# szcompressor/SZ3

Hardware: AMD Instinct MI355X
Metric: compression throughput GB/s + ratio at fixed abs errBound, 512^3 f32 (higher is better)
Workload: dtype f32; 1 GPU; C2: 3D float32 512x512x512 synthetic field per GPU, Lorenzo predictor, abs errBound=0.001, device-resident in -> device-resident Huffman payload; parallelism=slab1, algo=HIP_LORENZO(16), exchange=none (one rank)

## Files before the change

### include/sz3hip_debug.h

```cpp
#ifndef SZ3HIP_DEBUG_H
#define SZ3HIP_DEBUG_H

enum sz3hip_dbg {
    SZ3HIP_DBG_CB_COMPACT_IN_WG = 1,
    SZ3HIP_DBG_K1_LAB_NO_HIST = 1,
    SZ3HIP_DBG_DEC_MULTI_SYM = 2,
    SZ3HIP_DBG_K1_NO_CODE_STORES = 2,
    SZ3HIP_DBG_BLKDEC_FORCE_RETRY = 4,
    SZ3HIP_DBG_K1_V4_NO_STENCIL = 4,
    SZ3HIP_DBG_K1_NO_Q16 = 8,
    SZ3HIP_DBG_BLKDEC_LOCAL_EXPANDED = 16,
    SZ3HIP_DBG_K1_V4_NO_PREFETCH = 16,
    SZ3HIP_DBG_PACK_LAB_NO_STORES = 16,
    SZ3HIP_DBG_K1_NO_MARCH = 32,
    SZ3HIP_DBG_K1_NO_NARROW = 64,
    SZ3HIP_DBG_INTERP_NO_VEC = 128,
    SZ3HIP_DBG_K1_NO_WIDTH_SPEC = 256,
    SZ3HIP_DBG_DEC_NO_FUSED_X = 512,
    SZ3HIP_DBG_PACK_LAB_ONE_UNIT = 512,
    SZ3HIP_DBG_CB_ONE_CLASS = 1024,
    SZ3HIP_DBG_K1_NO_FUSED = 2048,
    SZ3HIP_DBG_BLK_RANK_3_LAUNCHES = 2048,
    SZ3HIP_DBG_BLK_SIDE_8_LAUNCHES = 2048,
    SZ3HIP_DBG_K1_NO_XCD_ORDER = 4096,
    SZ3HIP_DBG_CB_NO_SPEC_WIDE = 4096,
    SZ3HIP_DBG_INTERP_HIST_BIG = 8192,
    SZ3HIP_DBG_BLK_OFF = 16384,
    SZ3HIP_DBG_PACK_OLD = 32768,
    SZ3HIP_DBG_BLKDEC_GROUPS_3 = 32768,
    SZ3HIP_DBG_CB_NO_SAMPLED = 65536,
    SZ3HIP_DBG_BLKDEC_PER_FRONT = 65536,
    SZ3HIP_DBG_CTX_NO_MEMORY = 131072,
    SZ3HIP_DBG_CB_SERIAL_MERGE = 262144,
    SZ3HIP_DBG_DEC_NO_STORES = 524288,
    SZ3HIP_DBG_DEC_DIRECT_STORES = 1048576,
    SZ3HIP_DBG_DEC_NO_HALF = 2097152,
    SZ3HIP_DBG_INTERP_LEVELS_ANY_SIZE = 4194304,
    SZ3HIP_DBG_K1_NO_SAMP_IN_LAUNCH = 4194304,
    SZ3HIP_DBG_BLKDEC_BLOCK_PER_WAVE = 8388608,
    SZ3HIP_DBG_K1_Q16_PLAIN_STORES = 8388608,
    SZ3HIP_DBG_K1_NO_DEFER_FOLD = 16777216,
    SZ3HIP_DBG_PACK_NO_SEG_BITS = 33554432,
    SZ3HIP_DBG_BLK_FIT_TILES = 67108864,
    SZ3HIP_DBG_BLK_1D_WAVE_PER_BLOCK = 134217728,
    SZ3HIP_DBG_CTX_NO_PUBLISH_ZERO = 268435456,
    SZ3HIP_DBG_INTERP_HANDOVER_IN_PLACE = 536870912,
    SZ3HIP_DBG_DEC_CARRY_PASS = 536870912,
    SZ3HIP_DBG_BLK_NO_EXIT = 1073741824,
    SZ3HIP_DBG_BLK_NO_SELECT = -2147483647 - 1
};

enum sz3hip_dbg2 {
    SZ3HIP_DBG2_PACK_SCAN_LAUNCH = 1
};

#endif
```

### sz3_amd/__init__.py

```python
import contextlib
import ctypes as C
import enum
import os

import numpy as np

_HERE = os.path.dirname(os.path.abspath(__file__))
LIB_PATH = os.environ.get("SZ3HIP_LIB") or os.path.join(_HERE, "libsz3hip.so")

EB_ABS, EB_REL, EB_PSNR, EB_L2NORM, EB_ABS_AND_REL, EB_ABS_OR_REL = range(6)
ALGO_LORENZO_REG, ALGO_INTERP_LORENZO, ALGO_INTERP, ALGO_NOPRED, ALGO_LOSSLESS = range(5)
ALGO_HIP_LORENZO = 16
ALGO_HIP_INTERP = 17
INTERP_ALGO_LINEAR, INTERP_ALGO_CUBIC = 0, 1
SZ_FLOAT, SZ_DOUBLE = 0, 1


class Dbg(enum.IntFlag):
    CB_COMPACT_IN_WG = 1
    K1_LAB_NO_HIST = 1
    DEC_MULTI_SYM = 2
    K1_NO_CODE_STORES = 2
    BLKDEC_FORCE_RETRY = 4
    K1_V4_NO_STENCIL = 4
# ... 11 lines not shown
    K1_NO_FUSED = 2048
    BLK_RANK_3_LAUNCHES = 2048
    BLK_SIDE_8_LAUNCHES = 2048
    K1_NO_XCD_ORDER = 4096
    CB_NO_SPEC_WIDE = 4096
    INTERP_HIST_BIG = 8192
    BLK_OFF = 16384
    PACK_OLD = 32768
    BLKDEC_GROUPS_3 = 32768
    CB_NO_SAMPLED = 65536
    BLKDEC_PER_FRONT = 65536
    CTX_NO_MEMORY = 131072
    CB_SERIAL_MERGE = 262144
    DEC_NO_STORES = 524288
    DEC_DIRECT_STORES = 1048576
    DEC_NO_HALF = 2097152
    INTERP_LEVELS_ANY_SIZE = 4194304
    K1_NO_SAMP_IN_LAUNCH = 4194304
    BLKDEC_BLOCK_PER_WAVE = 8388608
    K1_Q16_PLAIN_STORES = 8388608
    K1_NO_DEFER_FOLD = 16777216
    PACK_NO_SEG_BITS = 33554432
    BLK_FIT_TILES = 67108864
    BLK_1D_WAVE_PER_BLOCK = 134217728
    CTX_NO_PUBLISH_ZERO = 268435456
    INTERP_HANDOVER_IN_PLACE = 536870912
    DEC_CARRY_PASS = 536870912
    BLK_NO_EXIT = 1073741824
    BLK_NO_SELECT = 2147483648


class Dbg2(enum.IntFlag):
    PACK_SCAN_LAUNCH = 1


class SZ3HipError(RuntimeError):
    def __init__(self, code, msg):
        super().__init__("sz3hip error %d: %s" % (code, msg))
        self.code = code


class _CConfig(C.Structure):
    _fields_ = [
        ("N", C.c_int32), ("dims", C.c_uint64 * 4), ("num", C.c_uint64),
        ("cmprAlgo", C.c_uint8), ("errorBoundMode", C.c_uint8),
        ("absErrorBound", C.c_double), ("relErrorBound", C.c_double),
        ("psnrErrorBound", C.c_double), ("l2normErrorBound", C.c_double),
        ("openmp", C.c_uint8), ("quantbinCnt", C.c_int32), ("blockSize", C.c_int32),
        ("predDim", C.c_uint8), ("dataType", C.c_uint8),
        ("lorenzo", C.c_uint8), ("lorenzo2", C.c_uint8), ("regression", C.c_uint8), ("regression2", C.c_uint8),
        ("interpAlgo", C.c_uint8), ("interpDirection", C.c_uint8),
        ("interpAnchorStride", C.c_int32), ("interpAlpha", C.c_double), ("interpBeta", C.c_double),
    ]


class _CTunerReport(C.Structure):
    _fields_ = [("ran", C.c_int32), ("use_interp", C.c_int32), ("sample_block_size", C.c_uint64), ("n_filtered", C.c_uint64),
                ("n_blocks", C.c_uint64), ("profiling", C.c_int32), ("interpAlgo", C.c_int32), ("interpDirection", C.c_int32),
                ("speculated", C.c_int32), ("interpAlpha", C.c_double), ("interpBeta", C.c_double), ("est_bytes", C.c_double * 8)]


class _CStats(C.Structure):
    _fields_ = [("n", C.c_uint64), ("n_value_outliers", C.c_uint64), ("n_delta_outliers", C.c_uint64),
                ("n_chunks", C.c_uint64), ("bitstream_bytes", C.c_uint64), ("payload_bytes", C.c_uint64),
                ("n_symbols", C.c_uint32), ("max_code_len", C.c_uint32),
                ("narrow_codes", C.c_uint32), ("reserved", C.c_uint32)]
# ... 992 lines not shown
```

### sz3_amd/csrc/sz3hip_kernels.h

```cpp
#ifndef SZ3HIP_KERNELS_H
#define SZ3HIP_KERNELS_H
#include <hip/hip_runtime.h>
#include <stdint.h>
#include "sz3hip_format.h"
#include "../../include/sz3hip_debug.h"

struct szk_lattice {
    double recip, two_eb, eb;
    float recip_f, two_eb_f, eb_lo_f;
};
static inline szk_lattice szk_make_lattice(double eb) {
    szk_lattice l;
    l.eb = eb;
    l.two_eb = 2.0 * eb;
    l.recip = 1.0 / l.two_eb;
    l.recip_f = (float)l.recip;
    l.two_eb_f = (float)l.two_eb;
    float e = (float)eb;
    if ((double)e > eb) e = __builtin_nextafterf(e, 0.0f);
    l.eb_lo_f = e;
    return l;
}

#define SZK_K1_GRID 2048u
// ... 6 lines not shown
    uint64_t n_total;
    uint32_t allow;
};

struct szk_cb_info;
#define SZK_SAMP_UNITS 1024u
#define SZK_SAMP_ROLES 128u
#define SZK_SAMP_MIN_ELEMS (1ull << 22)
#define SZK_SAMP_SEEN_LEN 16u
#define SZK_SAMP_WORDS 512u
#define SZK_SAMP_TICKET 320u
#define SZK_SAMP_LENS 384u
#define SZK_SAMP_READY 448u
struct szk_samp {
    uint32_t *words;
    uint32_t *enc;
    uint8_t *lens;
    szk_cb_info *info;
};
struct szk_k1_params {
    uint64_t d[4];
    szk_lattice lat;
    uint32_t radius;
    uint32_t dbg;
    szk_mode mode;
    uint64_t out_cap;
    uint64_t *hist;
    uint32_t *hist_partial;
    uint64_t *n_vout, *n_dout;
    uint64_t *vout_idx, *dout_idx;
    void *vout_val, *dout_val;
    void *prof_ev0, *prof_ev1;
    uint32_t wide16;
    uint32_t *range;
    int hint_narrow;
    const uint8_t *spec_lens;
    uint16_t *seg_bits;
    uint32_t *seg_made;
    int seg_expected;
    int assumed_narrow;
    int hint_q16;
    int assumed_q16;
    uint32_t *q16_flag;
    int defer_fold;
    uint32_t fold_rows;
    int range_kept;
    int fuse;
    int fused;
    const uint32_t *fuse_enc;
    const szk_cb_info *fuse_info;
    uint32_t *fuse_slots;
    uint64_t fuse_cap_words;
    uint32_t *seg_base;
    uint32_t *fuse_flag;
    uint32_t fuse_geom[4];
    szk_samp samp;
    int samp_in_launch;
};

struct szk_cb_info {
    uint32_t n_symbols, max_len, sym_min, sym_count;
    uint32_t win_lo, reserved;
    uint32_t esc_sym, pad0;
    uint64_t ts[12];
    uint32_t first_code[SZH_MAX_LEN + 2];
};
// ... 397 lines not shown
```

### sz3_amd/csrc/sz3hip_kernels.hip

```cpp
#include <hip/hip_runtime.h>
#include <cstddef>
#include <stdint.h>
#include <type_traits>
#include <mutex>
#include <utility>
#include <vector>
#include "sz3hip_format.h"
#include "sz3hip_kernels.h"

#include "sz3hip_devutil.h"

template <typename T>
__global__ __launch_bounds__(256) void k_minmax(const T *__restrict__ in, uint64_t n, double *partial) {
    double mn = INFINITY, mx = -INFINITY;
    bool has_nan = false;
    for (uint64_t i = (uint64_t)blockIdx.x * blockDim.x + threadIdx.x; i < n; i += (uint64_t)gridDim.x * blockDim.x) {
        double v = (double)in[i];
        if (v < mn) mn = v;
        if (v > mx) mx = v;
        has_nan |= (v != v);
    }
    (void)has_nan;
#pragma unroll
    for (int d = WAVE / 2; d > 0; d >>= 1) {
// ... 797 lines not shown
                if (MODE == 1 || MODE == 4) hist_add_ranged(p.hist, p.range, sym, (unsigned long long)v);
                else atomicAdd((unsigned long long *)&p.hist[sym], (unsigned long long)v);
            }
        }
    }
}

#define NARROW_BINS 256
template <typename T> struct NarrowCtx {
    using B = typename Lattice<T>::B;
    using OQV = typename std::conditional<sizeof(T) == 4, uint32_t, uint64_t>::type;
    const T *in;
    uint8_t *codes8;
    const szk_k1_params *p;
    uint32_t d0, d1, d2;
    uint64_t plane, vol;
    uint32_t *lh;
    const uint8_t *s_len;
    uint16_t *seg_bits;
    uint64_t *oq_idx;
    OQV *oq_val;
    uint32_t oq_n;
    int lane;
    const uint32_t *s_enc;
    uint32_t *stage;
    uint32_t *slot;
    uint32_t slot_base;
    uint32_t slot_w;
    uint32_t st_cnt;
    uint32_t *seg_base;
    const uint32_t *samp_words;
    uint32_t *s_have;
    uint32_t have_len;
};
#define FUSE_STAGE_WORDS(TY) ((TY) * 128 + 32 + 8)
static inline uint32_t fuse_slot_words(uint32_t ty, uint64_t d1, uint64_t d2) {
    return (uint32_t)((d1 < ty ? d1 : ty) * 128u * (d2 < MARCH_TZ ? d2 : MARCH_TZ) + 32u);
}
template <typename T>
__device__ __forceinline__ void narrow_oq_flush(NarrowCtx<T> &c) {
    c.oq_n = (uint32_t)__builtin_amdgcn_readfirstlane((int)c.oq_n);
    if (c.oq_n == 0) return;
    const szk_k1_params &p = *c.p;
    const unsigned long long act = __ballot(1);
    const uint32_t nact = (uint32_t)__popcll(act), rank = (uint32_t)__popcll(act & ((1ull << c.lane) - 1ull));
    unsigned long long base = 0;
    if (rank == 0) base = atomicAdd((unsigned long long *)p.n_vout, (unsigned long long)c.oq_n);
    const uint32_t blo = (uint32_t)__builtin_amdgcn_readfirstlane((int)(uint32_t)base);
    const uint32_t bhi = (uint32_t)__builtin_amdgcn_readfirstlane((int)(uint32_t)(base >> 32));
    const unsigned long long b0 = ((unsigned long long)bhi << 32) | blo;
    for (uint32_t k = rank; k < c.oq_n; k += nact) {
        const unsigned long long pos = b0 + k;
        if (pos < p.out_cap) {
            p.vout_idx[pos] = c.oq_idx[k];
            if (sizeof(T) == 4) reinterpret_cast<uint32_t *>(p.vout_val)[pos] = (uint32_t)c.oq_val[k];
            else reinterpret_cast<uint64_t *>(p.vout_val)[pos] = c.oq_val[k];
        }
    }
    c.oq_n = 0;
}
template <typename T>
__device__ __forceinline__ void narrow_rare(NarrowCtx<T> &c, uint64_t gi, const typename QTraits<T>::UQ (&delta)[4], uint32_t tmask, uint32_t badmask) {
    using Q = typename QTraits<T>::Q;
    using OQV = typename NarrowCtx<T>::OQV;
    const szk_k1_params &p = *c.p;
    constexpr uint32_t OQ = MarchLds<1, false>::OQ;
// ... 8 lines not shown
                }
                pd++;
            }
    }
#pragma unroll
    for (int i = 0; i < 4; i++) {
        const bool is_vout = (badmask >> i) & 1u;
        const unsigned long long vm = __ballot(is_vout);
        if (vm) {
            c.oq_n = (uint32_t)__builtin_amdgcn_readfirstlane((int)c.oq_n);
            if (c.oq_n + WAVE > OQ) narrow_oq_flush(c);
            if (is_vout) {
                const uint32_t slot = c.oq_n + (uint32_t)__popcll(vm & ((1ull << c.lane) - 1ull));
                c.oq_idx[slot] = gi + i;
                const T raw = c.in[gi + i];
                OQV bits = 0;
                memcpy(&bits, &raw, sizeof(T));
                c.oq_val[slot] = bits;
            }
            c.oq_n += (uint32_t)__popcll(vm);
        }
    }
    {
        const uint32_t cnt = (uint32_t)__popc(tmask & 15u);
        const unsigned long long b0 = __ballot(cnt & 1u), b1 = __ballot(cnt & 2u), b2 = __ballot(cnt & 4u), any = b0 | b1 | b2;
        if (any && c.lane == __ffsll((long long)any) - 1)
            hist_add_ranged(p.hist, p.range, 0u, (unsigned long long)(__popcll(b0) + 2 * __popcll(b1) + 4 * __popcll(b2)));
    }
}
template <typename T> __device__ __forceinline__ bool samp_take(const T *__restrict__ in, const szk_lattice &latp, uint32_t d0, uint32_t d1, uint32_t d2, uint32_t *words, uint32_t role, uint32_t *s_h);
__device__ __forceinline__ void samp_book(const szk_samp &sp, uint32_t radius, uint8_t *pool);
#define SAMP_POOL_BYTES (SZK_CB_SMALL_SYMS * 28 + 256)
template <typename T, typename PUT>
__device__ __forceinline__ bool samp_poll(NarrowCtx<T> &c, bool spin, PUT put) {
    volatile uint32_t *s_have = c.s_have;
    const uint32_t wv = (uint32_t)__builtin_amdgcn_readfirstlane((int)(threadIdx.x / WAVE));
    if (wv != 0) {
        uint32_t h = (uint32_t)__builtin_amdgcn_readfirstlane((int)*s_have);
        if (!h) {
            if (!spin) return false;
            do {
                __builtin_amdgcn_s_sleep(16);
                h = (uint32_t)__builtin_amdgcn_readfirstlane((int)*s_have);
            } while (!h);
        }
        __builtin_amdgcn_fence(__ATOMIC_ACQUIRE, "workgroup");
        c.have_len = 1;
        return true;
    }
    uint32_t r = __hip_atomic_load(const_cast<uint32_t *>(c.samp_words) + SZK_SAMP_READY, __ATOMIC_RELAXED, __HIP_MEMORY_SCOPE_AGENT);
    r = (uint32_t)__builtin_amdgcn_readfirstlane((int)r);
    if (!r) {
        if (!spin) return false;
        do {
            __builtin_amdgcn_s_sleep(32);
            r = __hip_atomic_load(const_cast<uint32_t *>(c.samp_words) + SZK_SAMP_READY, __ATOMIC_RELAXED, __HIP_MEMORY_SCOPE_AGENT);
            r = (uint32_t)__builtin_amdgcn_readfirstlane((int)r);
        } while (!r);
    }
    const uint32_t w = __hip_atomic_load(const_cast<uint32_t *>(c.samp_words) + SZK_SAMP_LENS + c.lane, __ATOMIC_RELAXED, __HIP_MEMORY_SCOPE_AGENT);
#pragma unroll
    for (int j = 0; j < 4; j++) put(4u * (uint32_t)c.lane + j, (w >> (8 * j)) & 0xFFu);
    __builtin_amdgcn_fence(__ATOMIC_RELEASE, "workgroup");
    __builtin_amdgcn_wave_barrier();
    if (c.lane == 0) *s_have = 1u;
    c.have_len = 1;
    return true;
}
template <typename T, int NW, int TY> struct NarrowPlane {
    Quad<T> rq[NW][TY + 1];
    T rl[NW][TY + 1];
    bool rok[NW][TY + 1];
};
template <typename T>
__device__ __forceinline__ void fuse_sweep(NarrowCtx<T> &c, uint32_t nw) {
    uint32_t *out = c.slot + c.slot_w;
    auto sweep = [&](uint32_t i) {
        const uint2 wv = *reinterpret_cast<const uint2 *>(&c.stage[i]);
        *reinterpret_cast<uint2 *>(&c.stage[i]) = make_uint2(0u, 0u);
#if defined(LAB_FUSE) && (LAB_FUSE & 32)
        *reinterpret_cast<unsigned long long *>(&out[i]) = (unsigned long long)wv.x | ((unsigned long long)wv.y << 32);
#else
        __builtin_nontemporal_store((unsigned long long)wv.x | ((unsigned long long)wv.y << 32), reinterpret_cast<unsigned long long *>(&out[i]));
#endif
    };
    const uint32_t i0 = 2u * (uint32_t)c.lane;
    if (i0 < nw) sweep(i0);
    if (i0 + 2u * WAVE < nw) sweep(i0 + 2u * WAVE);
    if (nw > 4u * WAVE)
        for (uint32_t i = i0 + 4u * WAVE; i < nw; i += 2u * WAVE) sweep(i);
}
template <typename T>
__device__ __forceinline__ void fuse_flush_lines(NarrowCtx<T> &c) {
#if defined(LAB_FUSE) && (LAB_FUSE & 4)
    const uint32_t nfl = 0;
    c.st_cnt &= 31u;
#else
    const uint32_t nfl = c.st_cnt & ~31u;
#endif
// ... 449 lines not shown
    for (int bnn = threadIdx.x; bnn < HIST_WIN; bnn += 256) {
        const int t = bnn - (HIST_WIN / 2 - 127);
        row[bnn] = (t >= 0 && t < 255) ? lh[t * 4] + lh[t * 4 + 1] + lh[t * 4 + 2] + lh[t * 4 + 3] : 0u;
    }
}

#define Q16_LIM 4095.0f
typedef float v2f32 __attribute__((ext_vector_type(2)));
typedef unsigned short v2u16 __attribute__((ext_vector_type(2)));
__device__ __forceinline__ uint32_t pk_sub16(uint32_t a, uint32_t b) {
    return __builtin_bit_cast(uint32_t, (v2u16)(__builtin_bit_cast(v2u16, a) - __builtin_bit_cast(v2u16, b)));
}
__device__ __forceinline__ uint32_t pk_add16(uint32_t a, uint32_t b) {
    return __builtin_bit_cast(uint32_t, (v2u16)(__builtin_bit_cast(v2u16, a) + __builtin_bit_cast(v2u16, b)));
}
__device__ __forceinline__ uint32_t pk_min16(uint32_t a, uint32_t b) {
    return __builtin_bit_cast(uint32_t, __builtin_elementwise_min(__builtin_bit_cast(v2u16, a), __builtin_bit_cast(v2u16, b)));
}
__device__ __forceinline__ uint32_t pk_max16(uint32_t a, uint32_t b) {
    return __builtin_bit_cast(uint32_t, __builtin_elementwise_max(__builtin_bit_cast(v2u16, a), __builtin_bit_cast(v2u16, b)));
}
__device__ __forceinline__ uint32_t pk_lo16(uint32_t a, uint32_t b) { return __builtin_amdgcn_perm(b, a, 0x05040100u); }
__device__ __forceinline__ uint32_t mad16_lo(uint32_t p, uint32_t add) {
    uint32_t d;
    asm("v_mad_u32_u16 %0, %1, 16, %2" : "=v"(d) : "v"(p), "v"(add));
    return d;
}
__device__ __forceinline__ uint32_t mad16_hi(uint32_t p, uint32_t add) {
    uint32_t d;
    asm("v_mad_u32_u16 %0, %1, 16, %2 op_sel:[1,0,0,0]" : "=v"(d) : "v"(p), "v"(add));
    return d;
}
#define Q16_LEN_OFF (NARROW_BINS * 16)
template <int TY> struct Q16Plane {
    float4 rq[TY + 1];
    float rl[TY + 1];
    bool rok[TY + 1];
};
template <int TY, bool EDGE, bool SAMP>
__device__ __forceinline__ void narrow16_task(NarrowCtx<float> &c, const Lattice<float> &lat, uint32_t *q16_flag, uint32_t x0, uint32_t y0, uint32_t z0) {
    const uint32_t d0 = c.d0, d1 = c.d1, d2 = c.d2;
    const int lane = c.lane;
    const uint32_t x = x0 + 4u * (uint32_t)lane;
    const bool xok = EDGE ? x < d0 : true;
    const uint32_t lane_off = xok ? x : 0u;
    const bool has_left = x0 > 0;
    const uint32_t c4 = ((uint32_t)lane & 3u) * 4u;
    uint8_t *const lds = reinterpret_cast<uint8_t *>(c.lh);
    const v2f32 recip2 = {lat.recip, lat.recip}, magic2 = {12582912.0f, 12582912.0f}, two_eb2 = {lat.two_eb, lat.two_eb};

    uint32_t ppA[TY], ppB[TY];
#pragma unroll
    for (int yy = 0; yy < TY; yy++) ppA[yy] = ppB[yy] = 0;

    auto fetch = [&](int zz, Q16Plane<TY> &R) {
        const float *src = c.in + (uint64_t)(z0 + (uint32_t)zz) * c.plane;
#pragma unroll
        for (int r = 0; r <= TY; r++) {
            const uint32_t gy = y0 + (uint32_t)r - 1u;
            R.rok[r] = gy < d1;
            if (R.rok[r]) {
                const float *row = src + (uint64_t)gy * d0;
#ifdef LAB_Q16_NTL
                {
                    typedef float f4v __attribute__((ext_vector_type(4)));
                    const f4v q = __builtin_nontemporal_load(reinterpret_cast<const f4v *>(row + lane_off));
                    R.rq[r] = make_float4(q.x, q.y, q.z, q.w);
                }
#else
                R.rq[r] = *reinterpret_cast<const float4 *>(row + lane_off);
#endif
                if (has_left) R.rl[r] = row[x0 - 1];
            }
        }
    };
    Q16Plane<TY> pa;
    auto work = [&](int zz, Q16Plane<TY> &R) {
        const uint32_t gz = z0 + (uint32_t)zz;
        uint32_t pd1A = 0, pd1B = 0;
        uint32_t bits_rows[(TY + 1) / 2];
#pragma unroll
        for (int k = 0; k < (TY + 1) / 2; k++) bits_rows[k] = 0;
        float qmax = 0.0f;
#pragma unroll
        for (int r = 0; r <= TY; r++) {
            uint32_t d1A = 0, d1B = 0;
            v2f32 s01 = {0.0f, 0.0f}, s23 = {0.0f, 0.0f}, t01 = magic2, t23 = magic2;
            if (R.rok[r]) {
                const v2f32 v01 = {R.rq[r].x, R.rq[r].y}, v23 = {R.rq[r].z, R.rq[r].w};
                s01 = v01 * recip2;
                s23 = v23 * recip2;
                t01 = s01 + magic2;
                t23 = s23 + magic2;
                uint32_t PA = pk_lo16(__float_as_uint(t01.x), __float_as_uint(t23.x));
                uint32_t PB = pk_lo16(__float_as_uint(t01.y), __float_as_uint(t23.y));
                if (EDGE) {
                    PA = xok ? PA : 0u;
                    PB = xok ? PB : 0u;
                }
                const uint32_t leftp = has_left ? __float_as_uint(R.rl[r] * lat.recip + 12582912.0f) << 16 : 0u;
                const uint32_t pv = (uint32_t)dpp_wave_shr1((int32_t)leftp, (int32_t)PB);
                const uint32_t XA = __builtin_amdgcn_alignbit(PB, pv, 16);
                d1A = pk_sub16(PA, XA);
                d1B = pk_sub16(PB, PA);
            }
            uint32_t sA = 0, sB = 0;
            if (r > 0) {
                const uint32_t d2A = pk_sub16(d1A, pd1A), d2B = pk_sub16(d1B, pd1B);
                sA = pk_sub16(d2A, ppA[r - 1]);
// ... 5 lines not shown
            pd1B = d1B;
            if (r == 0 || zz < 0) continue;
            if (!R.rok[r]) continue;
            const uint64_t grow = (uint64_t)gz * c.plane + (uint64_t)(y0 + r - 1) * d0;
            const uint32_t tqA = pk_add16(sA, 0x007F007Fu), tqB = pk_add16(sB, 0x007F007Fu);
            const uint32_t tA = pk_min16(tqA, 0x00FF00FFu), tB = pk_min16(tqB, 0x00FF00FFu);
            const uint32_t tm = pk_max16(tA, tB);
            const v2f32 r01 = t01 - magic2, r23 = t23 - magic2;
            const v2f32 v01 = {R.rq[r].x, R.rq[r].y}, v23 = {R.rq[r].z, R.rq[r].w};
            const v2f32 e01 = r01 * two_eb2 - v01, e23 = r23 * two_eb2 - v23;
            const bool b0 = !(fabsf(e01.x) <= lat.eb_lo), b1 = !(fabsf(e01.y) <= lat.eb_lo), b2 = !(fabsf(e23.x) <= lat.eb_lo), b3 = !(fabsf(e23.y) <= lat.eb_lo);
            qmax = fmaxf(fmaxf(qmax, fabsf(r01.x)), fabsf(r01.y));
            qmax = fmaxf(fmaxf(qmax, fabsf(r23.x)), fabsf(r23.y));
            bool rare = b0 | b1 | b2 | b3 | ((tm & 0xFFFFu) == 255u) | (tm >= 0x00FF0000u);
            if (EDGE) rare &= xok;
            const uint32_t a0 = mad16_lo(tA, c4), a1 = mad16_lo(tB, c4), a2 = mad16_hi(tA, c4), a3 = mad16_hi(tB, c4);
            if (!EDGE || xok) {
                if (!SAMP) {
                    atomicAdd(reinterpret_cast<uint32_t *>(lds + a0), 1u);
                    atomicAdd(reinterpret_cast<uint32_t *>(lds + a1), 1u);
                    atomicAdd(reinterpret_cast<uint32_t *>(lds + a2), 1u);
                    atomicAdd(reinterpret_cast<uint32_t *>(lds + a3), 1u);
                }
#if defined(LAB_ST) && LAB_ST == 1
                __hip_atomic_store(reinterpret_cast<uint32_t *>(c.codes8 + grow + x), tA | (tB << 8), __ATOMIC_RELAXED, __HIP_MEMORY_SCOPE_SYSTEM);
#elif defined(LAB_ST) && LAB_ST == 2
                *reinterpret_cast<uint32_t *>(c.codes8 + grow + x) = tA | (tB << 8);
#elif defined(LAB_ST) && LAB_ST == 3
                __hip_atomic_store(reinterpret_cast<uint32_t *>(c.codes8 + grow + x), tA | (tB << 8), __ATOMIC_RELAXED, __HIP_MEMORY_SCOPE_AGENT);
#else
                if (c.p->dbg & SZ3HIP_DBG_K1_Q16_PLAIN_STORES) *reinterpret_cast<uint32_t *>(c.codes8 + grow + x) = tA | (tB << 8);
                else __builtin_nontemporal_store(tA | (tB << 8), reinterpret_cast<uint32_t *>(c.codes8 + grow + x));
#endif
            }
            if (SAMP ? c.have_len != 0u : c.s_len != nullptr) {
                uint32_t b4 = (uint32_t)lds[Q16_LEN_OFF + a0] + lds[Q16_LEN_OFF + a1] + lds[Q16_LEN_OFF + a2] + lds[Q16_LEN_OFF + a3];
                if (EDGE) b4 = xok ? b4 : 0u;
                bits_rows[(r - 1) >> 1] |= ((r - 1) & 1) ? b4 << 16 : b4;
            }
            if (__builtin_amdgcn_ballot_w64(rare)) {
                const bool bad[4] = {b0, b1, b2, b3};
                const float sv[4] = {s01.x, s01.y, s23.x, s23.y};
                const uint32_t t[4] = {tA & 0xFFFFu, tB & 0xFFFFu, tA >> 16, tB >> 16};
                const uint32_t delta[4] = {(uint32_t)(int32_t)(int16_t)(sA & 0xFFFFu), (uint32_t)(int32_t)(int16_t)(sB & 0xFFFFu),
                                           (uint32_t)(int32_t)(int16_t)(sA >> 16), (uint32_t)(int32_t)(int16_t)(sB >> 16)};
                uint32_t tmask = 0, badmask = 0;
                bool alien = false;
#pragma unroll
                for (int i = 0; i < 4; i++) {
                    tmask |= (uint32_t)(rare && t[i] == 255u) << i;
                    badmask |= (uint32_t)(rare && bad[i]) << i;
                    alien |= rare && bad[i] && !(fabsf(sv[i]) <= 4194304.0f);
                }
                if (alien) atomicOr(q16_flag, 1u);
                narrow_rare<float>(c, grow + x, delta, tmask, badmask);
            }
        }
        if (zz >= 0) {
            bool big = !(qmax <= Q16_LIM);
            if (EDGE) big &= xok;
            if (__builtin_amdgcn_ballot_w64(big)) {
                if (big) atomicOr(q16_flag, 1u);
            }
        }
        if ((SAMP ? c.have_len != 0u : c.s_len != nullptr) && zz >= 0) {
#pragma unroll
            for (int k = 0; k < (TY + 1) / 2; k++) {
                const uint32_t tot = wave_sum(bits_rows[k]);
                const uint32_t ra = y0 + 2u * k, rb = ra + 1u;
                if (lane == 0) {
                    const uint64_t g0 = (uint64_t)gz * c.plane + x0;
                    if (ra < d1) c.seg_bits[(g0 + (uint64_t)ra * d0) >> 8] = (uint16_t)(tot & 0xFFFFu);
                    if (2 * k + 1 < TY && rb < d1) c.seg_bits[(g0 + (uint64_t)rb * d0) >> 8] = (uint16_t)(tot >> 16);
                }
            }
        }
    };
    int zz = z0 > 0 ? -1 : 0;
    const int zend = d2 - z0 < (uint32_t)MARCH_TZ ? (int)(d2 - z0) : MARCH_TZ;
    auto put_len = [&](uint32_t b, uint32_t len) {
        uint32_t *lt = c.lh + NARROW_BINS * 4 + b * 4u;
        lt[0] = lt[1] = lt[2] = lt[3] = len;
    };
    auto catch_up = [&](int zhi) __attribute__((always_inline)) {
        asm volatile("s_waitcnt vmcnt(0)" ::: "memory");
        constexpr int PB = 4;
        for (int p0 = 0; p0 < zhi; p0 += PB) {
            uint32_t cw[PB][TY];
#pragma unroll
            for (int j = 0; j < PB; j++) {
                const uint64_t gp = (uint64_t)(z0 + (uint32_t)(p0 + j)) * c.plane;
#pragma unroll
                for (int r = 0; r < TY; r++) {
                    const uint32_t ry = y0 + (uint32_t)r;
                    cw[j][r] = 0x80808080u;
                    if (p0 + j < zhi && ry < d1 && xok)
                        cw[j][r] = __hip_atomic_load(reinterpret_cast<uint32_t *>(c.codes8 + gp + (uint64_t)ry * d0 + x), __ATOMIC_RELAXED, __HIP_MEMORY_SCOPE_WORKGROUP);
                }
            }
#pragma unroll
            for (int j = 0; j < PB; j++) {
                const uint64_t gp = (uint64_t)(z0 + (uint32_t)(p0 + j)) * c.plane;
                if (p0 + j < zhi)
#pragma unroll
                for (int k = 0; k < (TY + 1) / 2; k++) {
                    uint32_t packed = 0;
#pragma unroll
                    for (int h = 0; h < 2; h++) {
                        const uint32_t ry = y0 + 2u * k + h;
                        if (2 * k + h < TY && ry < d1 && xok) {
                            const uint32_t w = cw[j][(2 * k + h) < TY ? 2 * k + h : 0];
                            const uint32_t b4 = (uint32_t)lds[Q16_LEN_OFF + (w & 0xFFu) * 16u + c4] + lds[Q16_LEN_OFF + ((w >> 8) & 0xFFu) * 16u + c4] +
                                                lds[Q16_LEN_OFF + ((w >> 16) & 0xFFu) * 16u + c4] + lds[Q16_LEN_OFF + (w >> 24) * 16u + c4];
                            packed |= h ? b4 << 16 : b4;
                        }
                    }
                    const uint32_t tot = wave_sum(packed);
                    const uint32_t ra = y0 + 2u * k, rb = ra + 1u;
                    if (lane == 0) {
                        const uint64_t g0 = gp + x0;
                        if (ra < d1) c.seg_bits[(g0 + (uint64_t)ra * d0) >> 8] = (uint16_t)(tot & 0xFFFFu);
                        if (2 * k + 1 < TY && rb < d1) c.seg_bits[(g0 + (uint64_t)rb * d0) >> 8] = (uint16_t)(tot >> 16);
                    }
                }
            }
        }
    };
    if (SAMP) {
        for (; zz < zend; zz++) {
            fetch(zz, pa);
            work(zz, pa);
            if (!c.have_len && zz >= 0 && samp_poll(c, false, put_len)) catch_up(zz + 1);
        }
        if (!c.have_len) {
            samp_poll(c, true, put_len);
            catch_up(zend);
        }
        return;
    }
#if defined(LAB_Q16PF) && LAB_Q16PF == 1
    Q16Plane<TY> pb;
    fetch(zz, pa);
    for (;;) {
        if (zz + 1 < zend) fetch(zz + 1, pb);
        work(zz, pa);
        if (++zz >= zend) break;
        if (zz + 1 < zend) fetch(zz + 1, pa);
        work(zz, pb);
        if (++zz >= zend) break;
    }
#else
    for (; zz < zend; zz++) {
        fetch(zz, pa);
        work(zz, pa);
    }
#endif
}
template <int TY, bool SAMP>
__device__ __forceinline__ void march_narrow16(const float *__restrict__ in, uint16_t *__restrict__ codes, const szk_k1_params &p, uint32_t ntasks,
                                               uint32_t *lh, uint64_t (*s_oq_idx)[MarchLds<1, false>::OQ], uint32_t (*s_oq_val)[MarchLds<1, false>::OQ]) {
    const Lattice<float> lat(p.lat);
    NarrowCtx<float> c;
    c.in = in;
    c.codes8 = reinterpret_cast<uint8_t *>(codes);
    c.p = &p;
    c.d0 = (uint32_t)p.d[3];
    c.d1 = (uint32_t)p.d[2];
    c.d2 = (uint32_t)p.d[1];
    c.plane = (uint64_t)c.d1 * c.d0;
    c.vol = c.plane * c.d2;
    c.lh = lh;
    c.lane = lane_id();
    const uint32_t wv = (uint32_t)__builtin_amdgcn_readfirstlane((int)(threadIdx.x / WAVE));
    c.oq_idx = s_oq_idx[wv];
    c.oq_val = s_oq_val[wv];
    c.oq_n = 0;
    const bool acct = SAMP || (p.spec_lens != nullptr && c.d0 % MARCH_TX == 0);
    c.s_len = acct ? reinterpret_cast<const uint8_t *>(lh) + Q16_LEN_OFF : nullptr;
    c.seg_bits = p.seg_bits;
    c.s_enc = nullptr;
    c.stage = nullptr;
    c.slot = nullptr;
    c.slot_w = c.slot_base = c.st_cnt = 0;
    c.seg_base = p.seg_base;
    c.samp_words = p.samp.words;
    c.s_have = lh + NARROW_BINS * 8;
    c.have_len = 0;
    const uint32_t bid = SAMP ? blockIdx.x - SZK_SAMP_ROLES : blockIdx.x, grid = SAMP ? gridDim.x - SZK_SAMP_ROLES : gridDim.x;
    for (int i = threadIdx.x; i < NARROW_BINS * 4; i += 256) lh[i] = 0;
    if (threadIdx.x == 0) lh[NARROW_BINS * 8] = 0;
    {
        const uint32_t b = threadIdx.x;
        const uint32_t len = (acct && !SAMP) ? p.spec_lens[b == 255u ? 0u : b + p.radius - 127u] : 0u;
#pragma unroll
        for (int k = 0; k < 4; k++) lh[NARROW_BINS * 4 + b * 4 + k] = len;
        if (acct && bid == 0 && threadIdx.x == 0) *p.seg_made = 1u;
    }
    __syncthreads();
    const uint32_t ntx = (c.d0 + MARCH_TX - 1) / MARCH_TX, nty = (c.d1 + TY - 1) / TY;
    const uint32_t per_xcd = grid / 8u;
    const uint32_t wg_seq = grid % 8u == 0 && !(p.dbg & SZ3HIP_DBG_K1_NO_XCD_ORDER) ? (bid % 8u) * per_xcd + bid / 8u : bid;
    const uint32_t nwaves = grid * 4u;
    for (uint32_t task = wg_seq * 4 + wv; task < ntasks; task += nwaves) {
        uint32_t b = task;
        const uint32_t x0 = (b % ntx) * MARCH_TX;
        b /= ntx;
        const uint32_t y0 = (b % nty) * TY;
        const uint32_t z0 = (b / nty) * MARCH_TZ;
        if (x0 + MARCH_TX <= c.d0 && y0 + TY <= c.d1) narrow16_task<TY, false, SAMP>(c, lat, p.q16_flag, x0, y0, z0);
        else narrow16_task<TY, true, SAMP>(c, lat, p.q16_flag, x0, y0, z0);
    }
    narrow_oq_flush(c);
    if (SAMP) return;
    __syncthreads();
    uint32_t *row = p.hist_partial + (uint64_t)blockIdx.x * HIST_WIN;
    for (int bnn = threadIdx.x; bnn < HIST_WIN; bnn += 256) {
        const int t = bnn - (HIST_WIN / 2 - 127);
        row[bnn] = (t >= 0 && t < 255) ? lh[t * 4] + lh[t * 4 + 1] + lh[t * 4 + 2] + lh[t * 4 + 3] : 0u;
    }
}
// ... 34 lines not shown
    __shared__ uint32_t s_p[4];
    if constexpr (SAMP) {
        static_assert(NDIM == 3, "1-D ... 3-D arrays");
        if (blockIdx.x < SZK_SAMP_ROLES) {
            if (blockIdx.x == 0 && threadIdx.x == 0) p.samp.info->ts[9] = wall_clock64();
            if (samp_take<T>(in, p.lat, (uint32_t)p.d[3], (uint32_t)p.d[2], (uint32_t)p.d[1], p.samp.words, blockIdx.x, lh)) samp_book(p.samp, p.radius, reinterpret_cast<uint8_t *>(lh));
            __syncthreads();
            probe_body<T, NDIM>(in, p, p.mode.n_total, p.mode.probe_big, s_p);
            return;
        }
    }
    probe_body<T, NDIM>(in, p, p.mode.n_total, p.mode.probe_big, s_p);
    march_narrow<T, NDIM, TY, false, SAMP>(in, codes, p, ntasks, lh, s_len, s_oq_idx, s_oq_val);
}
template <int TY, bool SAMP>
__global__ __launch_bounds__(256) void k_lorenzo_quant_march3q(const float *__restrict__ in, uint16_t *__restrict__ codes,
                                                               szk_k1_params p, uint32_t ntasks, uint32_t nrows) {
    using L = MarchLds<1, false>;
    __shared__ uint32_t lh[NARROW_BINS * 8 + 4];
    __shared__ uint64_t s_oq_idx[4][L::OQ];
    __shared__ uint32_t s_oq_val[4][L::OQ];
    __shared__ uint32_t s_p[4];
    if constexpr (SAMP) {
        static_assert(sizeof(lh) >= SAMP_POOL_BYTES && sizeof(lh) >= 4096, "the book's scratch fits the histogram");
        if (blockIdx.x < SZK_SAMP_ROLES) {
            if (blockIdx.x == 0 && threadIdx.x == 0) p.samp.info->ts[9] = wall_clock64();
            if (samp_take<float>(in, p.lat, (uint32_t)p.d[3], (uint32_t)p.d[2], (uint32_t)p.d[1], p.samp.words, blockIdx.x, lh)) samp_book(p.samp, p.radius, reinterpret_cast<uint8_t *>(lh));
            __syncthreads();
            probe_body<float, 3>(in, p, p.mode.n_total, p.mode.probe_big, s_p);
            return;
        }
    }
    probe_body<float, 3>(in, p, p.mode.n_total, p.mode.probe_big, s_p);
    march_narrow16<TY, SAMP>(in, codes, p, ntasks, lh, s_oq_idx, s_oq_val);
}
template <typename T, int NDIM, int TY>
__global__ __launch_bounds__(256) void k_lorenzo_quant_march3f(const T *__restrict__ in, uint16_t *__restrict__ codes,
                                                               szk_k1_params p, uint32_t ntasks, uint32_t nrows) {
    using L = MarchLds<1, false>;
    using OQV = typename std::conditional<sizeof(T) == 4, uint32_t, uint64_t>::type;
    __shared__ uint32_t lh[NARROW_BINS * 4 + 4];
    __shared__ uint64_t s_oq_idx[4][L::OQ];
    __shared__ OQV s_oq_val[4][L::OQ];
    __shared__ uint32_t s_p[4];
    __shared__ uint32_t s_fenc[256];
    __shared__ __align__(16) uint32_t s_fstage[4 * FUSE_STAGE_WORDS(TY)];
    probe_body<T, NDIM>(in, p, p.mode.n_total, p.mode.probe_big, s_p);
    march_narrow<T, NDIM, TY, true>(in, codes, p, ntasks, lh, nullptr, s_oq_idx, s_oq_val, s_fenc, s_fstage);
}

__global__ __launch_bounds__(256) void k_hist_reduce(const uint32_t *__restrict__ partial, uint32_t nrows, int win_lo,
                                                     uint64_t *__restrict__ hist, uint32_t *range) {
    const int bin = blockIdx.x * 256 + threadIdx.x;
    if (bin >= HIST_WIN) return;
    uint64_t s = 0;
    for (uint32_t r = blockIdx.y; r < nrows; r += gridDim.y) s += partial[(uint64_t)r * HIST_WIN + bin];
    const int sym = win_lo + bin;
    if (s && sym >= 0 && sym < (int)SZH_HIST_BINS) hist_add_ranged(hist, range, (uint32_t)sym, (unsigned long long)s);
}

#define CB_THREADS 256
#define CB_LAUNCH 1024
#define CB_LDS_SYMS 2048
#define CB_SMALL_SYMS SZK_CB_SMALL_SYMS
#define CB_POOL_BYTES 131072
#define CB_SHORT_SYMS 512
#define ENC_WIN 4096
// ... 4002 lines not shown
            if (fast) {
                launch_v4<T, 3, FTZ>(d_in, codes, p, tiles(64, 8, FTZ), s);
                break;
            }
            nb = tiles(64, 8, 8);
            if (nb > 0x7FFFFFFFull) return -1;
            hipLaunchKernelGGL((k_lorenzo_quant<T, 3, 64, 8, 8>), dim3((uint32_t)nb), dim3(256), 0, s, (const T *)d_in, codes, p);
            break;
        default:
            if (march) {
                launch_march<T, 4, MTY>(d_in, codes, p, one_launch, s);
                break;
            }
            if (fast) {
                launch_v4<T, 4, FTZ>(d_in, codes, p, tiles(64, 8, FTZ), s);
                break;
            }
            nb = tiles(64, 8, 4);
            if (nb > 0x7FFFFFFFull) return -1;
            hipLaunchKernelGGL((k_lorenzo_quant<T, 4, 64, 8, 4>), dim3((uint32_t)nb), dim3(256), 0, s, (const T *)d_in, codes, p);
            break;
    }
    SZK_CHECK_LAUNCH();
    return 0;
}
uint64_t szk_fuse_scratch_words(int ndim, const uint64_t d[4]) {
    if (ndim < 1 || ndim > 3 || d[3] % MARCH_TX != 0 || d[3] >= (1ull << 31) || d[2] >= (1ull << 31) || d[1] >= (1ull << 31)) return 0;
    const uint32_t ty = ndim == 1 ? 1u : (uint32_t)LAB_MTY;
    return march_tasks(d, ty) * fuse_slot_words(ty, d[2], d[1]) + 2;
}
int szk_launch_k1(int dtype, int ndim, const void *d_in, uint16_t *codes, szk_k1_params *p, hipStream_t s) {
    szk_k1_params &pp = *p;
    pp.dbg = (uint32_t)szk_dbg_flags;
    if (szk_dbg_flags & SZ3HIP_DBG_K1_NO_NARROW) pp.mode.allow = 0;
    return dtype == 0 ? launch_k1<float>(ndim, d_in, codes, pp, s) : launch_k1<double>(ndim, d_in, codes, pp, s);
}

int szk_launch_codebook(const uint64_t *d_hist, const szk_cb_params *p, hipStream_t s) {
    const uint32_t nb = p->n_books ? p->n_books : 1;
    szk_cb_params q = *p;
    q.n_books = nb;
    q.dbg = ((szk_dbg_flags & SZ3HIP_DBG_CB_ONE_CLASS) ? SZK_CB_DBG_ONE_CLASS : 0u) | ((szk_dbg_flags & SZ3HIP_DBG_CB_SERIAL_MERGE) ? SZK_CB_DBG_SERIAL_MERGE : 0u);
    if (nb > 1) {
        hipError_t e = hipMemsetAsync(q.range, 0, 16 * nb, s);
        if (e != hipSuccess) return (int)e;
    }
    if (!p->range_ready) hipLaunchKernelGGL(k_hist_range, dim3(SZH_HIST_BINS / 256, nb), dim3(256), 0, s, d_hist, q.range);
    q.keys_ready = nb == 1 && p->part_hint != 0 && !(szk_dbg_flags & SZ3HIP_DBG_CB_COMPACT_IN_WG) ? 1 : 0;
    if (q.keys_ready) hipLaunchKernelGGL(k_cb_compact, dim3(CBC_BLOCKS), dim3(1024), 0, s, d_hist, q.keys, q.syms, q.ifreq);
    if (p->part_hint != 1) hipLaunchKernelGGL(k_codebook<0>, dim3(nb == 1 ? 3 : nb), dim3(CB_LAUNCH), 0, s, d_hist, q);
    q.assign_later = q.keys_ready;
    if (p->part_hint != 0) hipLaunchKernelGGL(k_codebook<1>, dim3(nb == 1 ? 3 : nb), dim3(CB_LAUNCH), 0, s, d_hist, q);
    if (p->part_hint != 0 && q.assign_later) hipLaunchKernelGGL(k_cb_assign, dim3(16), dim3(1024), 0, s, (const uint16_t *)q.depth, (const uint16_t *)q.syms, (const szk_cb_info *)q.info, q.enc);
    SZK_CHECK_LAUNCH();
    return 0;
}
__global__ __launch_bounds__(1024) void k_book_verdict(const szk_cb_info *__restrict__ fresh, const uint8_t *__restrict__ fresh_lens,
                                                       const szk_cb_info *__restrict__ used, const uint8_t *__restrict__ used_lens,
                                                       const uint32_t *__restrict__ mispredict, const uint32_t *__restrict__ range, szk_state *state,
                                                       const uint64_t *__restrict__ hist, int exact) {
    __shared__ uint32_t s_diff;
    __shared__ unsigned long long s_acc[3];
    if (threadIdx.x == 0) s_diff = 0;
    if (threadIdx.x < 3) s_acc[threadIdx.x] = 0;
    __syncthreads();
    const bool built = *mispredict == 0;
// ... 396 lines not shown
```

Before: 2448 GB/s.

## Stash early Q16 code planes in LDS and split sample-ready poll around work

```diff
diff --git a/include/sz3hip_debug.h b/include/sz3hip_debug.h
--- a/include/sz3hip_debug.h
+++ b/include/sz3hip_debug.h
@@ -51,7 +51,10 @@
 };
 
 enum sz3hip_dbg2 {
-    SZ3HIP_DBG2_PACK_SCAN_LAUNCH = 1
+    SZ3HIP_DBG2_PACK_SCAN_LAUNCH = 1,
+    SZ3HIP_DBG2_K1_SAMP_NO_STASH = 2,
+    SZ3HIP_DBG2_K1_SAMP_STASH_ONE = 4,
+    SZ3HIP_DBG2_K1_SAMP_POLL_LATE = 8
 };
 
 #endif
diff --git a/sz3_amd/__init__.py b/sz3_amd/__init__.py
--- a/sz3_amd/__init__.py
+++ b/sz3_amd/__init__.py
@@ -67,6 +67,9 @@
 
 class Dbg2(enum.IntFlag):
     PACK_SCAN_LAUNCH = 1
+    K1_SAMP_NO_STASH = 2
+    K1_SAMP_STASH_ONE = 4
+    K1_SAMP_POLL_LATE = 8
 
 
 class SZ3HipError(RuntimeError):
diff --git a/sz3_amd/csrc/sz3hip_kernels.h b/sz3_amd/csrc/sz3hip_kernels.h
--- a/sz3_amd/csrc/sz3hip_kernels.h
+++ b/sz3_amd/csrc/sz3hip_kernels.h
@@ -62,6 +62,7 @@
     void *vout_val, *dout_val;
     void *prof_ev0, *prof_ev1;
     uint32_t wide16;
+    uint32_t dbg2;
     uint32_t *range;
     int hint_narrow;
     const uint8_t *spec_lens;
diff --git a/sz3_amd/csrc/sz3hip_kernels.hip b/sz3_amd/csrc/sz3hip_kernels.hip
--- a/sz3_amd/csrc/sz3hip_kernels.hip
+++ b/sz3_amd/csrc/sz3hip_kernels.hip
@@ -853,6 +853,7 @@
     const uint32_t *samp_words;
     uint32_t *s_have;
     uint32_t have_len;
+    uint32_t *stash;
 };
 #define FUSE_STAGE_WORDS(TY) ((TY) * 128 + 32 + 8)
 static inline uint32_t fuse_slot_words(uint32_t ty, uint64_t d1, uint64_t d2) {
@@ -927,6 +928,16 @@
 __device__ __forceinline__ void samp_book(const szk_samp &sp, uint32_t radius, uint8_t *pool);
 #define SAMP_POOL_BYTES (SZK_CB_SMALL_SYMS * 28 + 256)
 template <typename T, typename PUT>
+__device__ __forceinline__ void samp_fill(NarrowCtx<T> &c, PUT put) {
+    const uint32_t w = __hip_atomic_load(const_cast<uint32_t *>(c.samp_words) + SZK_SAMP_LENS + c.lane, __ATOMIC_RELAXED, __HIP_MEMORY_SCOPE_AGENT);
+#pragma unroll
+    for (int j = 0; j < 4; j++) put(4u * (uint32_t)c.lane + j, (w >> (8 * j)) & 0xFFu);
+    __builtin_amdgcn_fence(__ATOMIC_RELEASE, "workgroup");
+    __builtin_amdgcn_wave_barrier();
+    if (c.lane == 0) *(volatile uint32_t *)c.s_have = 1u;
+    c.have_len = 1;
+}
+template <typename T, typename PUT>
 __device__ __forceinline__ bool samp_poll(NarrowCtx<T> &c, bool spin, PUT put) {
     volatile uint32_t *s_have = c.s_have;
     const uint32_t wv = (uint32_t)__builtin_amdgcn_readfirstlane((int)(threadIdx.x / WAVE));
@@ -953,13 +964,23 @@
             r = (uint32_t)__builtin_amdgcn_readfirstlane((int)r);
         } while (!r);
     }
-    const uint32_t w = __hip_atomic_load(const_cast<uint32_t *>(c.samp_words) + SZK_SAMP_LENS + c.lane, __ATOMIC_RELAXED, __HIP_MEMORY_SCOPE_AGENT);
-#pragma unroll
-    for (int j = 0; j < 4; j++) put(4u * (uint32_t)c.lane + j, (w >> (8 * j)) & 0xFFu);
-    __builtin_amdgcn_fence(__ATOMIC_RELEASE, "workgroup");
-    __builtin_amdgcn_wave_barrier();
-    if (c.lane == 0) *s_have = 1u;
-    c.have_len = 1;
+    samp_fill(c, put);
+    return true;
+}
+__device__ __forceinline__ uint32_t samp_ask(const NarrowCtx<float> &c) {
+    return __hip_atomic_load(const_cast<uint32_t *>(c.samp_words) + SZK_SAMP_READY, __ATOMIC_RELAXED, __HIP_MEMORY_SCOPE_AGENT);
+}
+template <typename PUT>
+__device__ __forceinline__ bool samp_look(NarrowCtx<float> &c, uint32_t wv, uint32_t asked, PUT put) {
+    if (wv != 0) {
+        typedef __attribute__((address_space(3))) volatile uint32_t lds_word;
+        if (!__builtin_amdgcn_readfirstlane((int)*(lds_word *)c.s_have)) return false;
+        __builtin_amdgcn_fence(__ATOMIC_ACQUIRE, "workgroup");
+        c.have_len = 1;
+        return true;
+    }
+    if (!__builtin_amdgcn_readfirstlane((int)asked)) return false;
+    samp_fill(c, put);
     return true;
 }
 template <typename T, int NW, int TY> struct NarrowPlane {
@@ -1475,6 +1496,7 @@
     return d;
 }
 #define Q16_LEN_OFF (NARROW_BINS * 16)
+#define Q16_STASH_PLANES 4
 template <int TY> struct Q16Plane {
     float4 rq[TY + 1];
     float rl[TY + 1];
@@ -1518,6 +1540,10 @@
         }
     };
     Q16Plane<TY> pa;
+    auto stash_planes = [&]() -> int {
+        const uint32_t d = c.p->dbg2;
+        return (d & SZ3HIP_DBG2_K1_SAMP_NO_STASH) ? 0 : (d & SZ3HIP_DBG2_K1_SAMP_STASH_ONE) ? 1 : Q16_STASH_PLANES;
+    };
     auto work = [&](int zz, Q16Plane<TY> &R) {
         const uint32_t gz = z0 + (uint32_t)zz;
         uint32_t pd1A = 0, pd1B = 0;
@@ -1589,6 +1615,9 @@
                 if (c.p->dbg & SZ3HIP_DBG_K1_Q16_PLAIN_STORES) *reinterpret_cast<uint32_t *>(c.codes8 + grow + x) = tA | (tB << 8);
                 else __builtin_nontemporal_store(tA | (tB << 8), reinterpret_cast<uint32_t *>(c.codes8 + grow + x));
 #endif
+                if (SAMP) {
+                    if (!c.have_len && zz < stash_planes()) c.stash[(zz * TY + (r - 1)) * WAVE + lane] = tA | (tB << 8);
+                }
             }
             if (SAMP ? c.have_len != 0u : c.s_len != nullptr) {
                 uint32_t b4 = (uint32_t)lds[Q16_LEN_OFF + a0] + lds[Q16_LEN_OFF + a1] + lds[Q16_LEN_OFF + a2] + lds[Q16_LEN_OFF + a3];
@@ -1639,10 +1668,45 @@
         uint32_t *lt = c.lh + NARROW_BINS * 4 + b * 4u;
         lt[0] = lt[1] = lt[2] = lt[3] = len;
     };
+    auto plane_sums = [&](int pl, const uint32_t (&cw)[TY]) __attribute__((always_inline)) {
+        const uint64_t gp = (uint64_t)(z0 + (uint32_t)pl) * c.plane;
+#pragma unroll
+        for (int k = 0; k < (TY + 1) / 2; k++) {
+            uint32_t packed = 0;
+#pragma unroll
+            for (int h = 0; h < 2; h++) {
+                const uint32_t ry = y0 + 2u * k + h;
+                if (2 * k + h < TY && ry < d1 && xok) {
+                    const uint32_t w = cw[(2 * k + h) < TY ? 2 * k + h : 0];
+                    const uint32_t b4 = (uint32_t)lds[Q16_LEN_OFF + (w & 0xFFu) * 16u + c4] + lds[Q16_LEN_OFF + ((w >> 8) & 0xFFu) * 16u + c4] +
+                                        lds[Q16_LEN_OFF + ((w >> 16) & 0xFFu) * 16u + c4] + lds[Q16_LEN_OFF + (w >> 24) * 16u + c4];
+                    packed |= h ? b4 << 16 : b4;
+                }
+            }
+            const uint32_t tot = wave_sum(packed);
+            const uint32_t ra = y0 + 2u * k, rb = ra + 1u;
+            if (lane == 0) {
+                const uint64_t g0 = gp + x0;
+                if (ra < d1) c.seg_bits[(g0 + (uint64_t)ra * d0) >> 8] = (uint16_t)(tot & 0xFFFFu);
+                if (2 * k + 1 < TY && rb < d1) c.seg_bits[(g0 + (uint64_t)rb * d0) >> 8] = (uint16_t)(tot >> 16);
+            }
+        }
+    };
     auto catch_up = [&](int zhi) __attribute__((always_inline)) {
+        const int kst = stash_planes(), zst = zhi < kst ? zhi : kst;
+        for (int pl = 0; pl < zst; pl++) {
+            uint32_t cw[TY];
+#pragma unroll
+            for (int r = 0; r < TY; r++) {
+                cw[r] = 0x80808080u;
+                if (y0 + (uint32_t)r < d1 && xok) cw[r] = c.stash[(pl * TY + r) * WAVE + lane];
+            }
+            plane_sums(pl, cw);
+        }
+        if (zst >= zhi) return;
         asm volatile("s_waitcnt vmcnt(0)" ::: "memory");
         constexpr int PB = 4;
-        for (int p0 = 0; p0 < zhi; p0 += PB) {
+        for (int p0 = zst; p0 < zhi; p0 += PB) {
             uint32_t cw[PB][TY];
 #pragma unroll
             for (int j = 0; j < PB; j++) {
@@ -1656,38 +1720,19 @@
                 }
             }
 #pragma unroll
-            for (int j = 0; j < PB; j++) {
-                const uint64_t gp = (uint64_t)(z0 + (uint32_t)(p0 + j)) * c.plane;
-                if (p0 + j < zhi)
-#pragma unroll
-                for (int k = 0; k < (TY + 1) / 2; k++) {
-                    uint32_t packed = 0;
-#pragma unroll
-                    for (int h = 0; h < 2; h++) {
-                        const uint32_t ry = y0 + 2u * k + h;
-                        if (2 * k + h < TY && ry < d1 && xok) {
-                            const uint32_t w = cw[j][(2 * k + h) < TY ? 2 * k + h : 0];
-                            const uint32_t b4 = (uint32_t)lds[Q16_LEN_OFF + (w & 0xFFu) * 16u + c4] + lds[Q16_LEN_OFF + ((w >> 8) & 0xFFu) * 16u + c4] +
-                                                lds[Q16_LEN_OFF + ((w >> 16) & 0xFFu) * 16u + c4] + lds[Q16_LEN_OFF + (w >> 24) * 16u + c4];
-                            packed |= h ? b4 << 16 : b4;
-                        }
-                    }
-                    const uint32_t tot = wave_sum(packed);
-                    const uint32_t ra = y0 + 2u * k, rb = ra + 1u;
-                    if (lane == 0) {
-                        const uint64_t g0 = gp + x0;
-                        if (ra < d1) c.seg_bits[(g0 + (uint64_t)ra * d0) >> 8] = (uint16_t)(tot & 0xFFFFu);
-                        if (2 * k + 1 < TY && rb < d1) c.seg_bits[(g0 + (uint64_t)rb * d0) >> 8] = (uint16_t)(tot >> 16);
-                    }
-                }
-            }
+            for (int j = 0; j < PB; j++)
+                if (p0 + j < zhi) plane_sums(p0 + j, cw[j]);
         }
     };
     if (SAMP) {
+        const uint32_t wv = (uint32_t)__builtin_amdgcn_readfirstlane((int)(threadIdx.x / WAVE));
         for (; zz < zend; zz++) {
             fetch(zz, pa);
+            const bool look = !c.have_len && zz >= 0 && !(c.p->dbg2 & SZ3HIP_DBG2_K1_SAMP_POLL_LATE);
+            uint32_t asked = 0;
+            if (look && wv == 0) asked = samp_ask(c);
             work(zz, pa);
-            if (!c.have_len && zz >= 0 && samp_poll(c, false, put_len)) catch_up(zz + 1);
+            if (look && samp_look(c, wv, asked, put_len)) catch_up(zz + 1);
         }
         if (!c.have_len) {
             samp_poll(c, true, put_len);
@@ -1715,7 +1760,7 @@
 }
 template <int TY, bool SAMP>
 __device__ __forceinline__ void march_narrow16(const float *__restrict__ in, uint16_t *__restrict__ codes, const szk_k1_params &p, uint32_t ntasks,
-                                               uint32_t *lh, uint64_t (*s_oq_idx)[MarchLds<1, false>::OQ], uint32_t (*s_oq_val)[MarchLds<1, false>::OQ]) {
+                                               uint32_t *lh, uint64_t (*s_oq_idx)[MarchLds<1, false>::OQ], uint32_t (*s_oq_val)[MarchLds<1, false>::OQ], uint32_t *stash) {
     const Lattice<float> lat(p.lat);
     NarrowCtx<float> c;
     c.in = in;
@@ -1743,6 +1788,7 @@
     c.samp_words = p.samp.words;
     c.s_have = lh + NARROW_BINS * 8;
     c.have_len = 0;
+    c.stash = SAMP ? stash + wv * (Q16_STASH_PLANES * TY * WAVE) : nullptr;
     const uint32_t bid = SAMP ? blockIdx.x - SZK_SAMP_ROLES : blockIdx.x, grid = SAMP ? gridDim.x - SZK_SAMP_ROLES : gridDim.x;
     for (int i = threadIdx.x; i < NARROW_BINS * 4; i += 256) lh[i] = 0;
     if (threadIdx.x == 0) lh[NARROW_BINS * 8] = 0;
@@ -1843,7 +1889,13 @@
         }
     }
     probe_body<float, 3>(in, p, p.mode.n_total, p.mode.probe_big, s_p);
-    march_narrow16<TY, SAMP>(in, codes, p, ntasks, lh, s_oq_idx, s_oq_val);
+    if constexpr (SAMP) {
+        __shared__ uint32_t s_stash[4 * Q16_STASH_PLANES * TY * WAVE];
+        static_assert(sizeof(lh) + sizeof(s_oq_idx) + sizeof(s_oq_val) + sizeof(s_p) + sizeof(s_stash) <= 32768, "five workgroups per CU: the sampling workgroups and every worker resident at once");
+        march_narrow16<TY, SAMP>(in, codes, p, ntasks, lh, s_oq_idx, s_oq_val, s_stash);
+    } else {
+        march_narrow16<TY, SAMP>(in, codes, p, ntasks, lh, s_oq_idx, s_oq_val, nullptr);
+    }
 }
 template <typename T, int NDIM, int TY>
 __global__ __launch_bounds__(256) void k_lorenzo_quant_march3f(const T *__restrict__ in, uint16_t *__restrict__ codes,
@@ -5912,6 +5964,7 @@
 int szk_launch_k1(int dtype, int ndim, const void *d_in, uint16_t *codes, szk_k1_params *p, hipStream_t s) {
     szk_k1_params &pp = *p;
     pp.dbg = (uint32_t)szk_dbg_flags;
+    pp.dbg2 = (uint32_t)szk_dbg_flags2;
     if (szk_dbg_flags & SZ3HIP_DBG_K1_NO_NARROW) pp.mode.allow = 0;
     return dtype == 0 ? launch_k1<float>(ndim, d_in, codes, pp, s) : launch_k1<double>(ndim, d_in, codes, pp, s);
 }
```

New measurement: 2468 GB/s, median of 2. About the same (+0.8%).
